# NVIDIA-NeMo/NeMo

Hardware: AMD Instinct MI355X
Metric: audio-sec/s training throughput, Conformer-CTC-Large @ 1/2/4/8 MI355X (higher is better)
Workload: dtype bf16; 1 GPU; Conformer-CTC-Large bf16, batch=32x20s synthetic 16 kHz clips per GPU, 1xMI355X (BASELINE.json configs[1]); global_batch=32, parallelism=dp1

## Files before the change

include/mi355x_asr.h:

```cpp
#ifndef MI355X_ASR_H
#define MI355X_ASR_H
#ifdef __cplusplus
extern "C" {
#endif

#define MI355X_DT_F32 0
#define MI355X_DT_BF16 1

enum {
  MI355X_EPI_STORE = 0,
  MI355X_EPI_SWISH_DROP = 1,
  MI355X_EPI_RESID = 2,
  MI355X_EPI_DSWISH = 3,
  MI355X_EPI_RELU_MASK = 4,
  MI355X_EPI_MUL_POS = 5,
  MI355X_EPI_SWISH_DROP_G = 6,
  MI355X_EPI_DSWISH_G = 7
};
typedef struct mi355x_gemm_desc {
  const void* A; const void* B; void* C;
  int M, N, K;
  long long lda, ldb, ldc;
  long long c_col_stride;
  int transA, transB;
// ... 227 lines not shown

int mi355x_adamw_step(void* params, const void* grads, void* exp_avg, void* exp_avg_sq, long long n, float lr, float beta1,
                      float beta2, float eps, float weight_decay, int step, float grad_scale, void* stream);
int mi355x_adamw_step_ex(void* params, const void* grads, void* exp_avg, void* exp_avg_sq, long long n, float lr, float beta1,
                         float beta2, float eps, float weight_decay, int step, float grad_scale, const void* clip_coef,
                         void* ema, float ema_decay, void* stream);
int mi355x_grad_sumsq(const void* grads, long long n, void* out_f64, void* stream);
int mi355x_clip_coef(const void* sumsq_f64, int nbuf, float scale, float max_norm, void* coef_f32x2, void* stream);
typedef struct mi355x_pack_entry {
  const void* src; void* dst;
  int rows, cols, nr2, nc2;
  long long sr1, sr2, sc1, sc2, pitch;
  long long tile_begin;
} mi355x_pack_entry;
int mi355x_pack_weights(const void* table_dev, int n_entries, long long total_tiles, int out_dtype, void* stream);
int mi355x_fill_f32(void* p, long long n, float value, void* stream);

const char* mi355x_asr_version(void);

int mi355x_set_step_counter(const void* dev_word);
int mi355x_set_null_launch(int on);

int mi355x_stream_create(int priority, void** out_stream);
int mi355x_stream_destroy(void* stream);
typedef struct mi355x_tape mi355x_tape;
int mi355x_tape_log_begin(void* origin_stream);
int mi355x_tape_log_end(void);
int mi355x_tape_from_graph(void* hip_graph, int max_lanes, mi355x_tape** out);
int mi355x_tape_replay(mi355x_tape* tape, void* stream, int join);
int mi355x_tape_join(mi355x_tape* tape, void* stream);
// ... 132 lines not shown
```

nemo_amd/_lib.py:

```python
from __future__ import annotations

import ctypes as C
import os

import torch

_HERE = os.path.dirname(os.path.abspath(__file__))
LIB_PATH = os.environ.get("MI355X_ASR_LIB", os.path.join(_HERE, "lib", "libmi355x_asr.so"))

vp, i32, i64, f32, f64, u32 = C.c_void_p, C.c_int, C.c_longlong, C.c_float, C.c_double, C.c_uint


class GemmDesc(C.Structure):
    _fields_ = [
        ("A", vp), ("B", vp), ("C", vp),
        ("M", i32), ("N", i32), ("K", i32),
        ("lda", i64), ("ldb", i64), ("ldc", i64), ("c_col_stride", i64),
        ("transA", i32), ("transB", i32),
        ("in_dtype", i32), ("c_dtype", i32),
        ("batch", i32), ("nb0", i32),
        ("sA0", i64), ("sA1", i64), ("sB0", i64), ("sB1", i64), ("sC0", i64), ("sC1", i64),
        ("bias", vp), ("alpha", f32),
        ("epilogue", i32), ("atomic", i32), ("splitk", i32),
        ("aux_in", vp), ("aux_in_dtype", i32),
# ... 12 lines not shown


class RowMap(C.Structure):
    _fields_ = [("nI", i32), ("nJ", i32), ("OI", i32), ("OJ", i32), ("si", i32), ("sj", i32), ("oi", i32), ("oj", i32)]


class FfnPackEntry(C.Structure):
    _fields_ = [("src", vp), ("k512", vp), ("kchunk", vp), ("d_ff", i32), ("is_w2", i32)]


class PackEntry(C.Structure):
    _fields_ = [
        ("src", vp), ("dst", vp),
        ("rows", i32), ("cols", i32), ("nr2", i32), ("nc2", i32),
        ("sr1", i64), ("sr2", i64), ("sc1", i64), ("sc2", i64), ("pitch", i64),
        ("tile_begin", i64),
    ]


SIGNATURES = {
    "mi355x_gemm": [C.POINTER(GemmDesc), vp],
    "mi355x_gemm_grouped": [C.POINTER(GemmDesc), i32, vp],
    "mi355x_gemm_config": [i32, i32],
    "mi355x_gemm_plan": [C.POINTER(GemmDesc), C.POINTER(i32 * 8)],
    "mi355x_set_step_counter": [vp],
    "mi355x_set_null_launch": [i32],
    "mi355x_ffn_fwd": [vp, i64, vp, vp, vp, vp, vp, i64, vp, i64, vp, i64, i32, i32, i32, f32, u32, u32, f32, u32, u32, f32, vp],
    "mi355x_ffn_pack": [vp, i32, i32, vp],
    "mi355x_ffn_bwd_dgrad": [vp, i64, vp, vp, vp, i64, vp, vp, vp, i64, i32, i32, i32, u32, u32, f32, vp],
    "mi355x_logmel_fwd": [vp, vp, vp, i32, i32, i32, vp, vp, vp, vp, i32, f32, f32, u32, f32, vp, i32, i32, i32, vp],
# ... 70 lines not shown
    "mi355x_bn_finalize_dev_count": [vp, vp, vp, vp, vp, vp, f32, f32, i32, vp],
    "mi355x_bn_eval_stats": [vp, vp, vp, vp, f32, i32, vp],
    "mi355x_bn_swish_fwd": [vp, vp, vp, vp, vp, vp, i32, i64, i32, vp],
    "mi355x_bn_swish_bwd_reduce": [vp, vp, vp, vp, vp, vp, vp, vp, vp, i32, i64, i32, vp, i64, vp],
    "mi355x_bn_stats_swish_fwd": [vp, vp, f64, vp, vp, vp, vp, vp, vp, vp, vp, f32, f32, i32, i64, i32, vp],
    "mi355x_bn_swish_bwd_apply": [vp, vp, vp, vp, vp, vp, vp, f64, i32, vp, i32, i64, i32, vp],
    "mi355x_bn_swish_bwd_apply_dev_count": [vp, vp, vp, vp, vp, vp, vp, vp, i32, vp, i32, i64, i32, vp],
    "mi355x_bn_param_grad": [vp, vp, vp, i32, vp],
    "mi355x_ctc_loss": [vp, vp, vp, vp, vp, vp, vp, vp, i32, i32, i32, i32, i32, f32, i32, vp],
    "mi355x_row_scale": [vp, vp, i64, i64, vp],
    "mi355x_adamw_step": [vp, vp, vp, vp, i64, f32, f32, f32, f32, f32, i32, f32, vp],
    "mi355x_adamw_step_ex": [vp, vp, vp, vp, i64, f32, f32, f32, f32, f32, i32, f32, vp, vp, f32, vp],
    "mi355x_grad_sumsq": [vp, i64, vp, vp],
    "mi355x_clip_coef": [vp, i32, f32, f32, vp, vp],
    "mi355x_pack_weights": [vp, i32, i64, i32, vp],
    "mi355x_fill_f32": [vp, i64, f32, vp],
    "mi355x_rnnt_workspace_elems": [i32, i32, i32, vp],
    "mi355x_rnnt_loss": [vp, vp, vp, vp, i32, i32, i32, i32, i32, f32, f32, f32, vp, vp, vp, i64, vp],
    "mi355x_rnnt_greedy_decode": [vp, i32, i64, vp, vp, vp, i64, vp, i64, vp, vp, vp, i64, vp, vp, i64, vp, i32, i32, i32, i32, i32,
                                  i32, i32, i32, vp, vp, vp, vp, i32, vp, vp, vp],
    "mi355x_dwconv_config": [i32],
    "mi355x_ctc_config": [i32],
    "mi355x_ctc_align_config": [i32],
    "mi355x_logmel_config": [i32],
    "mi355x_stream_create": [i32, vp],
    "mi355x_stream_destroy": [vp],
    "mi355x_tape_log_begin": [vp],
    "mi355x_tape_log_end": [],
    "mi355x_tape_from_graph": [vp, i32, vp],
    "mi355x_tape_replay": [vp, vp, i32],
# ... 70 lines not shown
```

nemo_amd/csrc/optim.hip:

```cpp
#include "common.h"
#include "mi355x_asr.h"

__global__ __launch_bounds__(256) void adamw_kernel(float* __restrict__ p, const float* __restrict__ g, float* __restrict__ m,
                                                    float* __restrict__ v, long long n4, float lr, float beta1, float beta2,
                                                    float eps, float wd, float bc1, float bc2_sqrt, float grad_scale,
                                                    const float* __restrict__ gclip, float* __restrict__ ema, float ema_decay) {
  const float gs = gclip ? grad_scale * gclip[0] : grad_scale;
  for (long long i = blockIdx.x * 256LL + threadIdx.x; i < n4; i += (long long)gridDim.x * 256) {
    float pp[4], gg[4], mm[4], vv[4];
    ld4(p + i * 4, pp); ld4(g + i * 4, gg); ld4(m + i * 4, mm); ld4(v + i * 4, vv);
#pragma unroll
    for (int j = 0; j < 4; ++j) {
      const float gr = gg[j] * gs;
      pp[j] *= (1.f - lr * wd);
      mm[j] = beta1 * mm[j] + (1.f - beta1) * gr;
      vv[j] = beta2 * vv[j] + (1.f - beta2) * gr * gr;
      const float denom = sqrtf(vv[j]) / bc2_sqrt + eps;
      pp[j] -= (lr / bc1) * (mm[j] / denom);
    }
    st4(p + i * 4, pp); st4(m + i * 4, mm); st4(v + i * 4, vv);
    if (ema) {
      float ee[4];
      ld4(ema + i * 4, ee);
#pragma unroll
      for (int j = 0; j < 4; ++j) ee[j] = ee[j] * ema_decay + (1.f - ema_decay) * pp[j];
      st4(ema + i * 4, ee);
    }
  }
}
__global__ __launch_bounds__(256) void sumsq_kernel(const float* __restrict__ g, long long n4, double* __restrict__ out) {
  __shared__ float red[8];
  float a = 0.f;
  for (long long i = blockIdx.x * 256LL + threadIdx.x; i < n4; i += (long long)gridDim.x * 256) {
    float x[4];
    ld4(g + i * 4, x);
    a += (x[0] * x[0] + x[1] * x[1]) + (x[2] * x[2] + x[3] * x[3]);
  }
  a = block_sum(a, red);
  if (threadIdx.x == 0) atomicAdd(out, (double)a);
}
__global__ void clip_coef_kernel(const double* __restrict__ sumsq, int nbuf, float scale, float max_norm, float* __restrict__ coef) {
  double t = 0.0;
  for (int i = 0; i < nbuf; ++i) t += sumsq[i];
  const float norm = scale * (float)sqrt(t);
  const float c = max_norm / (norm + 1e-6f);
  coef[0] = c < 1.f ? c : 1.f;
  coef[1] = norm;
}

struct PackEntry {
  const float* src; void* dst;
  int rows, cols, nr2, nc2;
  long long sr1, sr2, sc1, sc2, pitch;
  long long tile_begin;
};
#define PK_T 64
__global__ __launch_bounds__(256) void pack_kernel(const PackEntry* __restrict__ tab, int n_entries, int out_dt) {
  __shared__ float tile[PK_T][PK_T + 1];
  int lo = 0, hi = n_entries - 1;
  const long long bid = blockIdx.x;
  while (lo < hi) {
    const int mid = (lo + hi + 1) >> 1;
    if (tab[mid].tile_begin <= bid) lo = mid; else hi = mid - 1;
  }
  const PackEntry e = tab[lo];
  const int tiles_c = (e.cols + PK_T - 1) / PK_T;
  const int local = (int)(bid - e.tile_begin);
  const int tr = local / tiles_c, tc = local - tr * tiles_c;
  const bool col_fast = (e.sc2 == 1 && e.nc2 > 1) || (e.nc2 == 1 && e.sc1 == 1);
  const bool plain = e.nr2 == 1 && e.nc2 == 1;
  const long long fast_stride = col_fast ? e.sc1 : e.sr1, slow_stride = col_fast ? e.sr1 : e.sc1;
// ... 68 lines not shown
}
extern "C" int mi355x_adamw_step(void* params, const void* grads, void* exp_avg, void* exp_avg_sq, long long n, float lr,
                                 float beta1, float beta2, float eps, float weight_decay, int step, float grad_scale,
                                 void* stream) {
  mi_clear_errors();
  return adamw_launch(params, grads, exp_avg, exp_avg_sq, n, lr, beta1, beta2, eps, weight_decay, step, grad_scale, nullptr,
                      nullptr, 0.f, stream);
}
extern "C" int mi355x_adamw_step_ex(void* params, const void* grads, void* exp_avg, void* exp_avg_sq, long long n, float lr,
                                    float beta1, float beta2, float eps, float weight_decay, int step, float grad_scale,
                                    const void* clip_coef, void* ema, float ema_decay, void* stream) {
  mi_clear_errors();
  return adamw_launch(params, grads, exp_avg, exp_avg_sq, n, lr, beta1, beta2, eps, weight_decay, step, grad_scale, clip_coef,
                      ema, ema_decay, stream);
}
extern "C" int mi355x_grad_sumsq(const void* grads, long long n, void* out_f64, void* stream) {
  mi_clear_errors();
  if (!grads || !out_f64 || n <= 0 || (n & 3)) return MI_ERR_ARG;
  long long nb = ((n >> 2) + 255) / 256;
  if (nb > 2048) nb = 2048;
  MI_LAUNCH(sumsq_kernel, dim3((unsigned)nb), dim3(256), 0, (hipStream_t)stream, (const float*)grads, n >> 2,
                     (double*)out_f64);
  return mi_check_launch();
}
extern "C" int mi355x_clip_coef(const void* sumsq_f64, int nbuf, float scale, float max_norm, void* coef_f32x2, void* stream) {
  mi_clear_errors();
  if (!sumsq_f64 || !coef_f32x2 || nbuf <= 0 || !(max_norm > 0.f)) return MI_ERR_ARG;
  MI_LAUNCH(clip_coef_kernel, dim3(1), dim3(1), 0, (hipStream_t)stream, (const double*)sumsq_f64, nbuf, scale, max_norm,
                     (float*)coef_f32x2);
  return mi_check_launch();
// ... 19 lines not shown
```

nemo_amd/flat.py:

```python
from __future__ import annotations

from typing import Dict, List, Tuple

import torch
from torch import nn

ALIGN = 64


class FlatParams:
    def __init__(self, module: nn.Module, tail=None):
        self.module = module
        self._tail = tail or (lambda name: False)
        self.flat: torch.Tensor = None
        self.grad: torch.Tensor = None
        self.offsets: Dict[str, Tuple[int, int]] = {}
        self.order: List[str] = []
        self.generation = 0

    def _params(self):
        ps = [(n, p) for n, p in self.module.named_parameters() if p.dtype == torch.float32]
        return [x for x in ps if not self._tail(x[0])] + [x for x in ps if self._tail(x[0])]

    def is_valid(self) -> bool:
        if self.flat is None:
            return False
        base, gbase = self.flat.data_ptr(), self.grad.data_ptr()
        for n, p in self._params():
            off = self.offsets.get(n)
            if off is None or p.data_ptr() != base + off[0] * 4:
                return False
            if p.grad is None or p.grad.data_ptr() != gbase + off[0] * 4:
                return False
# ... 12 lines not shown
            total += (p.numel() + ALIGN - 1) // ALIGN * ALIGN
        flat = torch.zeros(total, dtype=torch.float32, device=device)
        grad = torch.zeros(total, dtype=torch.float32, device=device)
        with torch.no_grad():
            for n, p in params:
                off, num = self.offsets[n]
                view = flat[off: off + num].view(p.shape)
                view.copy_(p.data.to(device))
                gview = grad[off: off + num].view(p.shape)
                if p.grad is not None:
                    gview.copy_(p.grad.to(device))
                p.data = view
                p.grad = gview
        self.flat, self.grad = flat, grad
        self.generation += 1

    def ensure(self, device=None) -> None:
        if not self.is_valid():
            self.build(device)

    def range_of(self, prefix: str) -> Tuple[int, int]:
        names = [n for n in self.order if n.startswith(prefix) and not self._tail(n)]
        if not names:
            raise KeyError(prefix)
        start = min(self.offsets[n][0] for n in names)
        end = max((self.offsets[n][0] + self.offsets[n][1] + ALIGN - 1) // ALIGN * ALIGN for n in names)
        return start, end

    def tail_range(self) -> Tuple[int, int]:
        names = [n for n in self.order if self._tail(n)]
# ... 33 lines not shown
```

nemo_amd/modules/conformer_encoder.py:

```python
from __future__ import annotations

import math
import os
from collections import OrderedDict
from typing import Any, NamedTuple, Optional

import torch
from torch import nn

from .. import ops
from ..core import (AcousticEncodedRepresentation, BoolType, ChannelType, LengthsType, NeuralModule, NeuralType, SpectrogramType,
                    typecheck)
from ..flat import FlatParams
from ..packing import PackPlan

INF_VAL = 10000.0


def _pad8(n):
    return (n + 7) // 8 * 8


class _FeedForward(nn.Module):
    def __init__(self, d_model, d_ff, use_bias=True):
# ... 337 lines not shown
        self._wg_pending, self._wg_rows = None, None
        self._defer_flush = None
        self.conv2_implicit = os.environ.get("MI355X_CONV2_IMPLICIT", "1") != "0"
        self.fuse_bn_dwconv_bwd = os.environ.get("MI355X_BN_DW_FUSE", "1") != "0"
        self.fuse_glu_dwconv_bwd = os.environ.get("MI355X_GLU_DW_FUSE", "1") != "0"
        self.tap_reduce_side = os.environ.get("MI355X_TAP_REDUCE_SIDE", "1") != "0"
        self.pad_tile_skip = os.environ.get("MI355X_PAD_SKIP", "1") != "0"
        self.fuse_glu_dwconv_fwd = os.environ.get("MI355X_GLU_DW_FUSE_FWD", "1") != "0"
        self.ln_cast_fuse = os.environ.get("MI355X_LN_CAST_FUSE", "1") != "0"
        self.ffn_fused = os.environ.get("MI355X_FFN_FUSED", "0") != "0"
        self.swish_g = os.environ.get("MI355X_SWISH_G", "1") != "0"
        self._saving = False
        self.dpos_side_stream = os.environ.get("MI355X_DPOS_STREAM", "1") != "0"
        self.sub_wgrad_side_stream = os.environ.get("MI355X_SUB_WGRAD_STREAM", "1") != "0"
        self._plans = {}
        self._ws = {}
        self._ws_retired = []
        self._pos_cache = {}
        self._step_seed = 0
        self._weights_version = -1
        self._token = None
        _g = os.environ.get("MI355X_GRAPHS", "auto")
        self.use_graphs = _g != "0"
        self.graph_auto = _g not in ("0", "1", "2")
        self.graph_tape = os.environ.get("MI355X_TAPE", "1") != "0"
        self.graph_bwd_live = os.environ.get("MI355X_GRAPHS_BWD_LIVE", "0") != "0"
        self.graph_warmup = 2
        self.graph_trials = 4
        self.max_graph_sets = int(os.environ.get("MI355X_GRAPH_SETS", "64"))
        self.graph_warmup_inherited = 1
# ... 13 lines not shown
        self._step_word = None

    def set_max_audio_length(self, max_audio_length):
        self.max_audio_length = max_audio_length

    def update_max_seq_length(self, seq_length: int, device):
        if seq_length > self.max_audio_length:
            self.set_max_audio_length(seq_length)

    def flat_parameters(self) -> FlatParams:
        self._flatp.ensure()
        return self._flatp

    def weights_updated(self):
        self._weights_version += 1

    def load_state_dict(self, *a, **k):
        r = super().load_state_dict(*a, **k)
        self.weights_updated()
        return r

    @staticmethod
    def _calc_att_context(att_context_size, att_context_probs, att_context_style):
        if att_context_style not in ("regular", "chunked_limited"):
            raise ValueError(f"att_context_style={att_context_style}")
        if att_context_size:
            all_ = [list(x) for x in ([att_context_size] if isinstance(list(att_context_size)[0], int) else list(att_context_size))]
            for i, cs in enumerate(all_):
                if att_context_style == "chunked_limited":
                    if cs[0] > 0 and cs[0] % (cs[1] + 1) > 0:
# ... 187 lines not shown

    def _buf(self, name, shape, dtype, device, zero=False):
        n = 1
        for k in shape:
            n *= int(k)
        key = (name, dtype)
        t = self._ws.get(key)
        if t is None or t.device != device or t.numel() < n:
            cap = n if t is None or t.device != device else max(n, int(t.numel() * 1.25))
            if t is not None:
                self._ws_retired.append(t)
            t = torch.zeros(cap, dtype=dtype, device=device) if zero else torch.empty(cap, dtype=dtype, device=device)
            self._ws[key] = t
        return t[:n].view(shape)

    def _plan(self, cdt, device):
        key = (cdt, str(device), self._flatp.generation, self._geometry(cdt))
        plan = self._plans.get(key)
        if plan is None:
            self._plans = {}
            p = PackPlan(cdt, device)
            pf = PackPlan(torch.float32, device)
            srcs = []
            pe = self.pre_encode
            C_, F2 = pe._conv_channels, pe._feat_after
            if self.subsampling == "striding":
                p.add_conv3x3("pre.w2", pe.conv[2].weight.data); p.add_conv3x3("pre.w2t", pe.conv[2].weight.data, transpose=True)
                w2flat = pe.conv[2].weight.data.view(-1)
                for par_t in (0, 1):
                    for par_f in (0, 1):
                        slots = self._dgrad_slots(par_t, par_f, pe._pad)
# ... 38 lines not shown
                            p.add_block(f"L{i}.att.wqkvt", w.view(-1)[h * dk * d_:], d_, dk, col_off=j * dA + h * dkp, sr1=1, sc1=d_)
                        p.add_block(f"L{i}.att.wpos", a.linear_pos.weight.data.view(-1)[h * dk * d_:], dk, d_, row_off=h * dkp,
                                    sr1=d_, sc1=1)
                        p.add_block(f"L{i}.att.wo", wo.view(-1)[h * dk:], d_, dk, col_off=h * dkp, sr1=d_, sc1=1)
                        p.add_block(f"L{i}.att.wot", wo.view(-1)[h * dk:], dk, d_, row_off=h * dkp, sr1=1, sc1=d_)
                        for j, b in enumerate((a.linear_q.bias.data, a.linear_k.bias.data, a.linear_v.bias.data)):
                            pf.add_block(f"L{i}.att.bqkv", b[h * dk:], 1, dk, col_off=j * dA + h * dkp, sr1=0, sc1=1)
                        pf.add_block(f"L{i}.att.bu", a.pos_bias_u.data.view(-1)[h * dk:], 1, dk, col_off=h * dkp, sr1=0, sc1=1)
                        pf.add_block(f"L{i}.att.bv", a.pos_bias_v.data.view(-1)[h * dk:], 1, dk, col_off=h * dkp, sr1=0, sc1=1)
                c = L.conv
                p.add_matrix(f"L{i}.conv.pw1", c.pointwise_conv1.weight.data); p.add_matrix(f"L{i}.conv.pw1t", c.pointwise_conv1.weight.data, True)
                p.add_matrix(f"L{i}.conv.pw2", c.pointwise_conv2.weight.data); p.add_matrix(f"L{i}.conv.pw2t", c.pointwise_conv2.weight.data, True)
            p.finalize(); pf.finalize()
            plan = (p, pf, None, -2)
            self._plans[key] = plan
        if plan[3] != self._weights_version or self._force_pack:
            plan[0].run(); plan[1].run()
            plan = (plan[0], plan[1], plan[2], self._weights_version)
            self._plans[key] = plan
        return plan[0], plan[1]

    def _eager_point(self, fn):
        if self._capture is None:
            fn()
        else:
            self._capture.cut(fn)

    def _hook(self, lo, hi):
        self._eager_point(lambda: self.grad_ready_hook(lo, hi) if self.grad_ready_hook is not None else None)

    def _graph_key(self, mel, length):
        return (tuple(mel.shape), self._cdt(), str(mel.device), self._flatp.generation, self._syncbn_world(),
                self.grad_ready_hook is not None, self._wgrad_join_per_layer, self.wgrad_side_stream, self.wgrad_grouped,
                self.dpos_side_stream, self.sub_wgrad_side_stream, self.conv2_implicit, self.ln_cast_fuse, self.fuse_bn_dwconv_bwd, self.fuse_glu_dwconv_bwd, self.fuse_glu_dwconv_fwd, self.tap_reduce_side, self.pad_tile_skip,
                self.use_flash_attention, self.flash_delta_residual, self.syncbn_profile is not None, self.graph_tape, self.swish_g, self.dropout, self.dropout_att, self.dropout_emb, self.dropout_pre_encoder,
# ... 55 lines not shown
            for k2, g2 in self._graph_sets.items():
                if g2 is not gs and g2.decided is not None and not g2.inherited and k2[1:] == key[1:]:
                    gs.decided, gs.inherited = g2.decided, True
                    gs.samples = {"eager": [], "graph": []}
                    if gs.decided == "eager":
                        gs.fwd = gs.bwd = gs.S = gs.out = gs.enc_len = gs.mel = gs.dout = None
                    break
        if auto and gs.decided is None and self._dp_world() > 1:
            gs.decided = "eager"
        if auto and (gs.decided == "eager" or not self._in_step):
            self.live_steps += 1
            return None
        if gs.failed or gs.calls <= (self.graph_warmup_inherited if gs.inherited else self.graph_warmup):
            self.live_steps += 1
            return None
        if gs.fwd is None:
            try:
                self._capture_forward(gs, mel, length)
            except Exception as e:
                if os.environ.get("MI355X_GRAPHS") == "2":
                    raise
                import warnings
                warnings.warn(f"recording the encoder forward as hipGraphs failed ({type(e).__name__}: {e}); this shape keeps "
                              "running on the eager sequencer")
                gs.failed, gs.fwd, gs.S = True, None, None
                self.live_steps += 1
                return None
        elif auto and gs.decided is None and gs.bwd is not None:
            n_e, n_g = len(gs.samples["eager"]), len(gs.samples["graph"])
            if n_e >= self.graph_trials and n_g >= self.graph_trials:
# ... 1232 lines not shown
```

nemo_amd/ops.py:

```python
from __future__ import annotations

import contextlib
import ctypes as C
from typing import Optional

import torch

from ._lib import ConvGather, GemmDesc, PackEntry, RowMap, check, lib

F32, BF16 = 0, 1
EPI_STORE, EPI_SWISH_DROP, EPI_RESID, EPI_DSWISH, EPI_RELU_MASK, EPI_MUL_POS, EPI_SWISH_DROP_G, EPI_DSWISH_G = range(8)

_DT = {torch.float32: F32, torch.bfloat16: BF16}


def dt(t) -> int:
    try:
        return _DT[t.dtype if isinstance(t, torch.Tensor) else t]
    except KeyError:
        raise ValueError(f"unsupported dtype {t.dtype if isinstance(t, torch.Tensor) else t}")


def _ptr(t: Optional[torch.Tensor]) -> int:
    if t is None:
# ... 804 lines not shown
def row_scale(x, vec, rows, cols):
    check(lib.mi355x_row_scale(_ptr(x), _ptr(vec), rows, cols, _stream()), "row_scale")


def adamw_step(params, grads, exp_avg, exp_avg_sq, lr, beta1, beta2, eps, weight_decay, step, grad_scale=1.0,
               clip_coef=None, ema=None, ema_decay=0.0):
    if clip_coef is None and ema is None:
        check(lib.mi355x_adamw_step(_ptr(params), _ptr(grads), _ptr(exp_avg), _ptr(exp_avg_sq), params.numel(), lr, beta1,
                                    beta2, eps, weight_decay, step, grad_scale, _stream()), "adamw_step")
    else:
        check(lib.mi355x_adamw_step_ex(_ptr(params), _ptr(grads), _ptr(exp_avg), _ptr(exp_avg_sq), params.numel(), lr, beta1,
                                       beta2, eps, weight_decay, step, grad_scale, _ptr(clip_coef), _ptr(ema), ema_decay,
                                       _stream()), "adamw_step_ex")


def grad_sumsq(grads, out_f64):
    check(lib.mi355x_grad_sumsq(_ptr(grads), grads.numel(), _ptr(out_f64), _stream()), "grad_sumsq")


def clip_coef(sumsq_f64, scale, max_norm, coef):
    check(lib.mi355x_clip_coef(_ptr(sumsq_f64), int(sumsq_f64.numel()), float(scale), float(max_norm), _ptr(coef), _stream()),
          "clip_coef")



def pack_weights(table_dev, n_entries, total_tiles, out_dtype):
    check(lib.mi355x_pack_weights(_ptr(table_dev), n_entries, total_tiles, out_dtype, _stream()), "pack_weights")


def fill_f32(t, value=0.0):
# ... 19 lines not shown
```

nemo_amd/optim.py:

```python
from __future__ import annotations

from typing import List

import torch

from . import ops
import math

from .flat import FlatParams


class NoamAnnealing:
    def __init__(self, base_lr: float, d_model: int, warmup_steps=None, warmup_ratio=None, max_steps=None, min_lr=0.0):
        assert not (warmup_steps is not None and warmup_ratio is not None), "Either use particular number of step or ratio"
        assert warmup_ratio is None or max_steps is not None, "If there is a ratio, there should be a total steps"
        if base_lr < min_lr:
            raise ValueError("initial learning rate lower than the minimum learning rate")
        self._normalize = d_model ** (-0.5)
        self.base_lr, self.min_lr = base_lr, min_lr
        self.warmup_steps = warmup_steps if warmup_steps is not None else (int(warmup_ratio * max_steps) if warmup_ratio else 0)
        self.last_epoch = 0

    def lr_at(self, step: int) -> float:
        step = max(1, step)
# ... 130 lines not shown
    def _ema_of(self, fp: FlatParams):
        if self.ema_decay is None:
            return None
        key = (id(fp), fp.generation)
        e = self._ema.get(key)
        if e is None:
            old = [v for k, v in self._ema.items() if k[0] == id(fp)]
            if old and old[0].numel() == fp.flat.numel():
                e = old[0].to(fp.flat.device)
            else:
                e = fp.flat.detach().clone()
            self._ema = {k: v for k, v in self._ema.items() if k[0] != id(fp)}
            self._ema[key] = e
        return e

    def zero_grad(self):
        for fp in self.flats:
            fp.ensure()
            fp.zero_grad()

    def begin_step(self, lr: float = None, grad_scale: float = 1.0):
        self.step_count += 1
        self._cur = (self.lr if lr is None else lr, grad_scale)
        self._done = {id(fp): [] for fp in self.flats}
        for fp in self.flats:
            fp.ensure()
            self._moments(fp)
            self._ema_of(fp)
        return self.max_grad_norm is None

    def step_range(self, fp: FlatParams, lo: int, hi: int):
        if getattr(self, "_cur", None) is None or self.max_grad_norm is not None or hi <= lo:
            return
        lr, grad_scale = self._cur
        m, v = self._moments(fp)
        ema = self._ema_of(fp)
        for tlo, thi in fp.trainable_ranges():
            a, b = max(lo, tlo), min(hi, thi)
            if a >= b:
                continue
            ops.adamw_step(fp.flat[a:b], fp.grad[a:b], m[a:b], v[a:b], lr, self.betas[0], self.betas[1], self.eps,
                           self.weight_decay, self.step_count, grad_scale, ema=None if ema is None else ema[a:b],
                           ema_decay=self.ema_decay or 0.0)
        self._done[id(fp)].append((lo, hi))

    def finish_step(self):
        lr, grad_scale = self._cur
        for fp in self.flats:
            done = sorted(self._done[id(fp)])
            pos, rest = 0, []
            for lo, hi in done:
                if lo > pos:
                    rest.append((pos, lo))
                pos = max(pos, hi)
            if pos < fp.flat.numel():
                rest.append((pos, fp.flat.numel()))
            for lo, hi in rest:
                self.step_range(fp, lo, hi)
        self._cur = None
        for fp in self.flats:
            if hasattr(fp.module, "weights_updated"):
                fp.module.weights_updated()

    def step(self, lr: float = None, grad_scale: float = 1.0):
        self.step_count += 1
        lr = self.lr if lr is None else lr
        coef = None
        if self.max_grad_norm:
            dev = self.flats[0].flat.device
            if self._clip is None or self._clip[0].device != dev:
                self._clip = (torch.zeros(len(self.flats), dtype=torch.float64, device=dev),
                              torch.zeros(2, dtype=torch.float32, device=dev))
            sumsq, coef = self._clip
            sumsq.zero_()
            for i, fp in enumerate(self.flats):
                for lo, hi in fp.trainable_ranges():
                    ops.grad_sumsq(fp.grad[lo:hi], sumsq[i:i + 1])
            ops.clip_coef(sumsq, grad_scale, self.max_grad_norm, coef)
            self.last_grad_norm = coef[1:2]
        for fp in self.flats:
            m, v = self._moments(fp)
            ema = self._ema_of(fp)
            for lo, hi in fp.trainable_ranges():
                ops.adamw_step(fp.flat[lo:hi], fp.grad[lo:hi], m[lo:hi], v[lo:hi], lr, self.betas[0], self.betas[1], self.eps,
                               self.weight_decay, self.step_count, grad_scale, clip_coef=coef,
                               ema=None if ema is None else ema[lo:hi], ema_decay=self.ema_decay or 0.0)
        for fp in self.flats:
            if hasattr(fp.module, "weights_updated"):
                fp.module.weights_updated()

    def swap_ema_weights(self):
        import contextlib

        @contextlib.contextmanager
        def ctx():
            if self.ema_decay is None:
                yield
                return
            pairs = [(fp, self._ema_of(fp)) for fp in self.flats]

            def swap():
# ... 31 lines not shown
```

nemo_amd/packing.py:

```python
from __future__ import annotations

import ctypes as C
from typing import Dict, List, Tuple

import numpy as np
import torch

from . import ops
from ._lib import PackEntry


def _pad8(n: int) -> int:
    return (n + 7) // 8 * 8


class PackPlan:
    def __init__(self, dtype: torch.dtype, device):
        self.dtype = dtype
        self.device = torch.device(device)
        self._images: Dict[str, Tuple[int, int, int]] = {}
        self._pending: List[tuple] = []
        self._size = 0
        self.arena = None
        self._table = None
        self._n = 0
        self._tiles = 0
        self._views: Dict[str, torch.Tensor] = {}
        self._ffn: List[tuple] = []
        self._ffn_table = None

    def new_image(self, name: str, rows: int, cols: int) -> None:
        pitch = _pad8(cols)
        self._images[name] = (self._size, rows, pitch)
        self._size += (rows * pitch + 63) // 64 * 64

    def add_block(self, name: str, src: torch.Tensor, rows: int, cols: int, *, row_off=0, col_off=0, nr2=1, nc2=1,
                  sr1=0, sr2=0, sc1=0, sc2=0) -> None:
        assert src.dtype == torch.float32 and src.is_contiguous()
        self._pending.append((name, src, rows, cols, row_off, col_off, nr2, nc2, sr1, sr2, sc1, sc2))

    def add_matrix(self, name: str, w: torch.Tensor, transpose: bool = False):
        R, Cc = w.shape[0], int(np.prod(w.shape[1:]))
        if not transpose:
            self.new_image(name, R, Cc)
# ... 40 lines not shown
            self.add_block(name, w, F_ * C_, d, nr2=C_, nc2=1, sr1=1, sr2=F_, sc1=C_ * F_)
        return name

    def add_ffn(self, prefix: str, w1: torch.Tensor, w2: torch.Tensor) -> None:
        dff = w1.shape[0]
        assert self.dtype == torch.bfloat16 and tuple(w1.shape) == (dff, 512) and tuple(w2.shape) == (512, dff) and dff % 64 == 0
        assert w1.dtype == torch.float32 and w2.dtype == torch.float32 and w1.is_contiguous() and w2.is_contiguous()
        for nm in ("w1p", "w1tp", "w2p", "w2tp"):
            self.new_image(f"{prefix}.{nm}", dff // 2, 1024)
        self._ffn.append((prefix, w1, w2, dff))

    def finalize(self) -> None:
        self.arena = torch.zeros(max(self._size, 64), dtype=self.dtype, device=self.device)
        es = self.arena.element_size()
        base = self.arena.data_ptr()
        entries = (PackEntry * len(self._pending))()
        tiles = 0
        for i, (name, src, rows, cols, ro, co, nr2, nc2, sr1, sr2, sc1, sc2) in enumerate(self._pending):
            off, irows, pitch = self._images[name]
            assert ro + rows <= irows and co + cols <= pitch, name
            e = entries[i]
            e.src = src.data_ptr()
            assert co % 8 == 0, name
            e.dst = base + (off + ro * pitch + co) * es
            e.rows, e.cols, e.nr2, e.nc2 = rows, cols, nr2, nc2
            e.sr1, e.sr2, e.sc1, e.sc2, e.pitch = sr1, sr2, sc1, sc2, pitch
            e.tile_begin = tiles
            tiles += ((rows + 63) // 64) * ((cols + 63) // 64)
        raw = bytes(entries)
        self._table = torch.frombuffer(bytearray(raw), dtype=torch.uint8).to(self.device) if raw else None
        self._n, self._tiles = len(self._pending), tiles
        self._srcs = [p[1] for p in self._pending]
        if self._ffn:
            from ._lib import FfnPackEntry
            fe = (FfnPackEntry * (2 * len(self._ffn)))()
            for i, (prefix, w1, w2, dff) in enumerate(self._ffn):
                off = {nm: self._images[f"{prefix}.{nm}"][0] for nm in ("w1p", "w1tp", "w2p", "w2tp")}
                a, b = fe[2 * i], fe[2 * i + 1]
                a.src, a.k512, a.kchunk, a.d_ff, a.is_w2 = w1.data_ptr(), base + off["w1p"] * es, base + off["w1tp"] * es, dff, 0
                b.src, b.k512, b.kchunk, b.d_ff, b.is_w2 = w2.data_ptr(), base + off["w2tp"] * es, base + off["w2p"] * es, dff, 1
            self._ffn_table = torch.frombuffer(bytearray(bytes(fe)), dtype=torch.uint8).to(self.device)
            self._srcs += [t for f in self._ffn for t in (f[1], f[2])]
        for name, (off, rows, pitch) in self._images.items():
            self._views[name] = self.arena[off: off + rows * pitch].view(rows, pitch)

    def source_ptrs(self):
        return [s.data_ptr() for s in self._srcs]

    def run(self) -> None:
        if self._n:
            ops.pack_weights(self._table, self._n, self._tiles, ops.dt(self.dtype))
        if self._ffn:
            ops.ffn_pack(self._ffn_table, 2 * len(self._ffn), max(f[3] for f in self._ffn))

    def __getitem__(self, name: str) -> torch.Tensor:
        return self._views[name]

    def pitch(self, name: str) -> int:
        return self._images[name][2]
```

Measured before the change: 18280 audio-sec/s.

## Fuse AdamW update with bf16 weight packing for plain matrix parameters

Adds a fused AdamW kernel that updates fp32 parameters and also writes the bf16 packed weight images (plain or transposed) for simple matrix parameters straight from the updated values. The separate pack pass then only handles the remaining entries. Bookkeeping tracks whether every covered matrix was handled by the fused path, with a catch-up pack when it was not. The aim is to save a separate read of the fp32 weights and a kernel launch per step. The cost is more complex cross-module state tracking and transposed stores that are not coalesced.

```diff
diff --git a/include/mi355x_asr.h b/include/mi355x_asr.h
--- a/include/mi355x_asr.h
+++ b/include/mi355x_asr.h
@@ -265,6 +265,18 @@
   long long tile_begin;
 } mi355x_pack_entry;
 int mi355x_pack_weights(const void* table_dev, int n_entries, long long total_tiles, int out_dtype, void* stream);
+typedef struct mi355x_adamw_pack_entry {
+  long long off;
+  int rows, cols;
+  void* dst0; void* dst1;
+  long long pitch0, pitch1;
+  int trans0, trans1;
+  long long tile_begin;
+} mi355x_adamw_pack_entry;
+int mi355x_adamw_pack_step(const void* table_dev, int n_entries, long long tile_base, long long n_tiles, void* params,
+                           const void* grads, void* exp_avg, void* exp_avg_sq, long long lo, long long hi, float lr, float beta1,
+                           float beta2, float eps, float weight_decay, int step, float grad_scale, const void* clip_coef,
+                           void* ema, float ema_decay, void* stream);
 int mi355x_fill_f32(void* p, long long n, float value, void* stream);
 
 const char* mi355x_asr_version(void);
diff --git a/nemo_amd/_lib.py b/nemo_amd/_lib.py
--- a/nemo_amd/_lib.py
+++ b/nemo_amd/_lib.py
@@ -50,6 +50,15 @@
         ("src", vp), ("dst", vp),
         ("rows", i32), ("cols", i32), ("nr2", i32), ("nc2", i32),
         ("sr1", i64), ("sr2", i64), ("sc1", i64), ("sc2", i64), ("pitch", i64),
+        ("tile_begin", i64),
+    ]
+
+
+class AdamwPackEntry(C.Structure):
+    _fields_ = [
+        ("off", i64), ("rows", i32), ("cols", i32),
+        ("dst0", vp), ("dst1", vp), ("pitch0", i64), ("pitch1", i64),
+        ("trans0", i32), ("trans1", i32),
         ("tile_begin", i64),
     ]
 
@@ -150,6 +159,7 @@
     "mi355x_grad_sumsq": [vp, i64, vp, vp],
     "mi355x_clip_coef": [vp, i32, f32, f32, vp, vp],
     "mi355x_pack_weights": [vp, i32, i64, i32, vp],
+    "mi355x_adamw_pack_step": [vp, i32, i64, i64, vp, vp, vp, vp, i64, i64, f32, f32, f32, f32, f32, i32, f32, vp, vp, f32, vp],
     "mi355x_fill_f32": [vp, i64, f32, vp],
     "mi355x_rnnt_workspace_elems": [i32, i32, i32, vp],
     "mi355x_rnnt_loss": [vp, vp, vp, vp, i32, i32, i32, i32, i32, f32, f32, f32, vp, vp, vp, i64, vp],
diff --git a/nemo_amd/csrc/optim.hip b/nemo_amd/csrc/optim.hip
--- a/nemo_amd/csrc/optim.hip
+++ b/nemo_amd/csrc/optim.hip
@@ -1,30 +1,146 @@
 #include "common.h"
 #include "mi355x_asr.h"
+
+#define PK_T 64
+struct AdamwC { float lr, beta1, beta2, eps, wd, bc1, bc2_sqrt, gs; };
+__device__ __forceinline__ void adamw_update(float& pp, const float gg, float& mm, float& vv, const AdamwC& c) {
+  const float gr = gg * c.gs;
+  mm = __builtin_fmaf(c.beta1, mm, (1.f - c.beta1) * gr);
+  vv = __builtin_fmaf(c.beta2, vv, gr * ((1.f - c.beta2) * gr));
+  const float denom = sqrtf(vv) / c.bc2_sqrt + c.eps;
+  const float upd = -(c.lr / c.bc1) * (mm / denom);
+  pp = __builtin_fmaf(__builtin_fmaf(-c.lr, c.wd, 1.f), pp, upd);
+}
+__device__ __forceinline__ float ema_update(const float ee, const float pp, const float ema_decay) {
+  return __builtin_fmaf(ema_decay, ee, (1.f - ema_decay) * pp);
+}
+__device__ __forceinline__ void adamw_compute4(float (&pp)[4], const float (&gg)[4], float (&mm)[4], float (&vv)[4],
+                                               const AdamwC& c) {
+#pragma unroll
+  for (int j = 0; j < 4; ++j) adamw_update(pp[j], gg[j], mm[j], vv[j], c);
+}
+__device__ __forceinline__ void adamw_update4(float* __restrict__ p, const float* __restrict__ g, float* __restrict__ m,
+                                              float* __restrict__ v, float* __restrict__ ema, float ema_decay, long long i,
+                                              const AdamwC& c, float (&pp)[4]) {
+  float gg[4], mm[4], vv[4];
+  ld4(p + i, pp); ld4(g + i, gg); ld4(m + i, mm); ld4(v + i, vv);
+  adamw_compute4(pp, gg, mm, vv, c);
+  st4(p + i, pp); st4(m + i, mm); st4(v + i, vv);
+  if (ema) {
+    float ee[4];
+    ld4(ema + i, ee);
+#pragma unroll
+    for (int j = 0; j < 4; ++j) ee[j] = ema_update(ee[j], pp[j], ema_decay);
+    st4(ema + i, ee);
+  }
+}
 
 __global__ __launch_bounds__(256) void adamw_kernel(float* __restrict__ p, const float* __restrict__ g, float* __restrict__ m,
                                                     float* __restrict__ v, long long n4, float lr, float beta1, float beta2,
                                                     float eps, float wd, float bc1, float bc2_sqrt, float grad_scale,
                                                     const float* __restrict__ gclip, float* __restrict__ ema, float ema_decay) {
-  const float gs = gclip ? grad_scale * gclip[0] : grad_scale;
+  const AdamwC c = {lr, beta1, beta2, eps, wd, bc1, bc2_sqrt, gclip ? grad_scale * gclip[0] : grad_scale};
   for (long long i = blockIdx.x * 256LL + threadIdx.x; i < n4; i += (long long)gridDim.x * 256) {
-    float pp[4], gg[4], mm[4], vv[4];
-    ld4(p + i * 4, pp); ld4(g + i * 4, gg); ld4(m + i * 4, mm); ld4(v + i * 4, vv);
-#pragma unroll
-    for (int j = 0; j < 4; ++j) {
-      const float gr = gg[j] * gs;
-      pp[j] *= (1.f - lr * wd);
-      mm[j] = beta1 * mm[j] + (1.f - beta1) * gr;
-      vv[j] = beta2 * vv[j] + (1.f - beta2) * gr * gr;
-      const float denom = sqrtf(vv[j]) / bc2_sqrt + eps;
-      pp[j] -= (lr / bc1) * (mm[j] / denom);
-    }
-    st4(p + i * 4, pp); st4(m + i * 4, mm); st4(v + i * 4, vv);
-    if (ema) {
-      float ee[4];
-      ld4(ema + i * 4, ee);
-#pragma unroll
-      for (int j = 0; j < 4; ++j) ee[j] = ee[j] * ema_decay + (1.f - ema_decay) * pp[j];
-      st4(ema + i * 4, ee);
+    float pp[4];
+    adamw_update4(p, g, m, v, ema, ema_decay, i * 4, c, pp);
+  }
+}
+
+#define APK_CHUNK 4096
+typedef mi355x_adamw_pack_entry AdamwPackEntry;
+__global__ __launch_bounds__(256) void adamw_pack_kernel(const AdamwPackEntry* __restrict__ tab, int n_entries, long long tile_base,
+                                                         float* __restrict__ p, const float* __restrict__ g,
+                                                         float* __restrict__ m, float* __restrict__ v, long long lo_el,
+                                                         long long hi_el, float lr, float beta1, float beta2, float eps, float wd,
+                                                         float bc1, float bc2_sqrt, float grad_scale,
+                                                         const float* __restrict__ gclip, float* __restrict__ ema,
+                                                         float ema_decay) {
+  const AdamwC c = {lr, beta1, beta2, eps, wd, bc1, bc2_sqrt, gclip ? grad_scale * gclip[0] : grad_scale};
+  int lo = 0, hi = n_entries - 1;
+  const long long bid = tile_base + blockIdx.x;
+  while (lo < hi) {
+    const int mid = (lo + hi + 1) >> 1;
+    if (tab[mid].tile_begin <= bid) lo = mid; else hi = mid - 1;
+  }
+  const AdamwPackEntry e = tab[lo];
+  const int local = (int)(bid - e.tile_begin);
+  if (e.rows == 0) {
+    long long a = e.off + (long long)local * APK_CHUNK, b = a + APK_CHUNK;
+    if (b > e.off + e.cols) b = e.off + e.cols;
+    if (a < lo_el) a = lo_el;
+    if (b > hi_el) b = hi_el;
+    for (long long i = a + threadIdx.x * 4; i < b; i += 256 * 4) {
+      float pp[4];
+      adamw_update4(p, g, m, v, ema, ema_decay, i, c, pp);
+    }
+    return;
+  }
+  const int tiles_c = (e.cols + PK_T - 1) / PK_T;
+  const int tr = local / tiles_c, tc = local - tr * tiles_c;
+  const int rb = tr * PK_T + (threadIdx.x >> 4) * 4, cc = tc * PK_T + (threadIdx.x & 15) * 4;
+  const bool vec = !(e.cols & 3);
+  float np[4][4];
+#pragma unroll
+  for (int k = 0; k < 4; ++k) {
+    const int r = rb + k;
+    const int nv = (r < e.rows && cc < e.cols) ? (e.cols - cc < 4 ? e.cols - cc : 4) : 0;
+    const bool whole = vec && nv == 4;
+    const long long i = e.off + (long long)r * e.cols + cc;
+    float pp[4] = {0.f, 0.f, 0.f, 0.f}, gg[4] = {0.f, 0.f, 0.f, 0.f}, mm[4] = {0.f, 0.f, 0.f, 0.f}, vv[4] = {0.f, 0.f, 0.f, 0.f};
+    float ee[4] = {0.f, 0.f, 0.f, 0.f};
+    if (whole) {
+      ld4(p + i, pp); ld4(g + i, gg); ld4(m + i, mm); ld4(v + i, vv);
+      if (ema) ld4(ema + i, ee);
+    } else {
+#pragma unroll
+      for (int j = 0; j < 4; ++j)
+        if (j < nv) {
+          pp[j] = p[i + j]; gg[j] = g[i + j]; mm[j] = m[i + j]; vv[j] = v[i + j];
+          if (ema) ee[j] = ema[i + j];
+        }
+    }
+    adamw_compute4(pp, gg, mm, vv, c);
+#pragma unroll
+    for (int j = 0; j < 4; ++j) ee[j] = ema_update(ee[j], pp[j], ema_decay);
+    if (whole) {
+      st4(p + i, pp); st4(m + i, mm); st4(v + i, vv);
+      if (ema) st4(ema + i, ee);
+    } else {
+#pragma unroll
+      for (int j = 0; j < 4; ++j) {
+        if (j < nv) {
+          p[i + j] = pp[j]; m[i + j] = mm[j]; v[i + j] = vv[j];
+          if (ema) ema[i + j] = ee[j];
+        } else {
+          pp[j] = 0.f;
+        }
+      }
+    }
+#pragma unroll
+    for (int j = 0; j < 4; ++j) np[k][j] = pp[j];
+  }
+  const int rows8 = (e.rows + 7) & ~7, cols8 = (e.cols + 7) & ~7;
+#pragma unroll
+  for (int d = 0; d < 2; ++d) {
+    bf16_t* dst = (bf16_t*)(d ? e.dst1 : e.dst0);
+    if (!dst) continue;
+    const long long pitch = d ? e.pitch1 : e.pitch0;
+    if (!(d ? e.trans1 : e.trans0)) {
+      if (cc < cols8) {
+#pragma unroll
+        for (int k = 0; k < 4; ++k)
+          if (rb + k < e.rows)
+            *reinterpret_cast<uint2*>(dst + (long long)(rb + k) * pitch + cc) =
+                make_uint2(pack_bf2(np[k][0], np[k][1]), pack_bf2(np[k][2], np[k][3]));
+      }
+    } else {
+      if (rb < rows8) {
+#pragma unroll
+        for (int j = 0; j < 4; ++j)
+          if (cc + j < e.cols)
+            *reinterpret_cast<uint2*>(dst + (long long)(cc + j) * pitch + rb) =
+                make_uint2(pack_bf2(np[0][j], np[1][j]), pack_bf2(np[2][j], np[3][j]));
+      }
     }
   }
 }
@@ -54,7 +170,6 @@
   long long sr1, sr2, sc1, sc2, pitch;
   long long tile_begin;
 };
-#define PK_T 64
 __global__ __launch_bounds__(256) void pack_kernel(const PackEntry* __restrict__ tab, int n_entries, int out_dt) {
   __shared__ float tile[PK_T][PK_T + 1];
   int lo = 0, hi = n_entries - 1;
@@ -153,6 +268,21 @@
   return adamw_launch(params, grads, exp_avg, exp_avg_sq, n, lr, beta1, beta2, eps, weight_decay, step, grad_scale, clip_coef,
                       ema, ema_decay, stream);
 }
+extern "C" int mi355x_adamw_pack_step(const void* table_dev, int n_entries, long long tile_base, long long n_tiles, void* params,
+                                      const void* grads, void* exp_avg, void* exp_avg_sq, long long lo, long long hi, float lr,
+                                      float beta1, float beta2, float eps, float weight_decay, int step, float grad_scale,
+                                      const void* clip_coef, void* ema, float ema_decay, void* stream) {
+  mi_clear_errors();
+  if (!table_dev || n_entries <= 0 || tile_base < 0 || n_tiles <= 0 || n_tiles > 0x7fffffffLL) return MI_ERR_ARG;
+  if (!params || !grads || !exp_avg || !exp_avg_sq || lo < 0 || hi <= lo || (lo & 3) || (hi & 3) || step < 1) return MI_ERR_ARG;
+  if (ema && !(ema_decay >= 0.f && ema_decay <= 1.f)) return MI_ERR_ARG;
+  const float bc1 = 1.f - powf(beta1, (float)step);
+  const float bc2s = sqrtf(1.f - powf(beta2, (float)step));
+  MI_LAUNCH(adamw_pack_kernel, dim3((unsigned)n_tiles), dim3(256), 0, (hipStream_t)stream, (const AdamwPackEntry*)table_dev,
+                     n_entries, tile_base, (float*)params, (const float*)grads, (float*)exp_avg, (float*)exp_avg_sq, lo, hi, lr,
+                     beta1, beta2, eps, weight_decay, bc1, bc2s, grad_scale, (const float*)clip_coef, (float*)ema, ema_decay);
+  return mi_check_launch();
+}
 extern "C" int mi355x_grad_sumsq(const void* grads, long long n, void* out_f64, void* stream) {
   mi_clear_errors();
   if (!grads || !out_f64 || n <= 0 || (n & 3)) return MI_ERR_ARG;
diff --git a/nemo_amd/flat.py b/nemo_amd/flat.py
--- a/nemo_amd/flat.py
+++ b/nemo_amd/flat.py
@@ -17,6 +17,19 @@
         self.offsets: Dict[str, Tuple[int, int]] = {}
         self.order: List[str] = []
         self.generation = 0
+        self.fused_table = None
+
+    def set_fused_table(self, table) -> None:
+        self.fused_table = table
+
+    def fused(self):
+        t = self.fused_table
+        return t if t is not None and t.matches(self) else None
+
+    def fused_lookup(self, lo: int, hi: int):
+        t = self.fused()
+        sub = t.lookup(lo, hi) if t is not None else None
+        return None if sub is None else (t, sub)
 
     def _params(self):
         ps = [(n, p) for n, p in self.module.named_parameters() if p.dtype == torch.float32]
@@ -59,6 +72,7 @@
                 p.grad = gview
         self.flat, self.grad = flat, grad
         self.generation += 1
+        self.fused_table = None
 
     def ensure(self, device=None) -> None:
         if not self.is_valid():
diff --git a/nemo_amd/modules/conformer_encoder.py b/nemo_amd/modules/conformer_encoder.py
--- a/nemo_amd/modules/conformer_encoder.py
+++ b/nemo_amd/modules/conformer_encoder.py
@@ -375,6 +375,7 @@
         self.dpos_side_stream = os.environ.get("MI355X_DPOS_STREAM", "1") != "0"
         self.sub_wgrad_side_stream = os.environ.get("MI355X_SUB_WGRAD_STREAM", "1") != "0"
         self._plans = {}
+        self.adamw_pack = os.environ.get("MI355X_ADAMW_PACK", "1") != "0"
         self._ws = {}
         self._ws_retired = []
         self._pos_cache = {}
@@ -418,6 +419,9 @@
 
     def weights_updated(self):
         self._weights_version += 1
+        tab = self._flatp.fused_table
+        if tab is not None:
+            tab.plan.covered_at = self._weights_version if tab.take_complete() else None
 
     def load_state_dict(self, *a, **k):
         r = super().load_state_dict(*a, **k)
@@ -635,7 +639,7 @@
             self._ws[key] = t
         return t[:n].view(shape)
 
-    def _plan(self, cdt, device):
+    def _plan(self, cdt, device, pack=True):
         key = (cdt, str(device), self._flatp.generation, self._geometry(cdt))
         plan = self._plans.get(key)
         if plan is None:
@@ -704,11 +708,33 @@
             p.finalize(); pf.finalize()
             plan = (p, pf, None, -2)
             self._plans[key] = plan
+            fused_ok = cdt == torch.bfloat16 and self._flatp.flat.device == p.arena.device
+            self._flatp.set_fused_table(p.build_fused(self._flatp) if fused_ok else None)
+        if plan[0].fused is not None:
+            plan[0].fused.enabled = self.adamw_pack
+        if not pack:
+            return plan[0], plan[1]
         if plan[3] != self._weights_version or self._force_pack:
-            plan[0].run(); plan[1].run()
+            p = plan[0]
+            rest_only = p.fused is not None and p.covered_at == self._weights_version
+            p.run(rest_only=rest_only); plan[1].run()
+            if p.fused is not None:
+                p.covered_at = self._weights_version
             plan = (plan[0], plan[1], plan[2], self._weights_version)
             self._plans[key] = plan
         return plan[0], plan[1]
+
+    def _covered_catch_up(self, cdt, device):
+        plan = self._plans.get((cdt, str(device), self._flatp.generation, self._geometry(cdt)))
+        if plan is None:
+            return
+        p = plan[0]
+        if p.fused is None:
+            return
+        p.fused.enabled = self.adamw_pack
+        if p.covered_at != self._weights_version:
+            p.run(covered_only=True)
+            p.covered_at = self._weights_version
 
     def _eager_point(self, fn):
         if self._capture is None:
@@ -794,6 +820,7 @@
         if gs.failed or gs.calls <= (self.graph_warmup_inherited if gs.inherited else self.graph_warmup):
             self.live_steps += 1
             return None
+        self._covered_catch_up(self._cdt(), mel.device)
         if gs.fwd is None:
             try:
                 self._capture_forward(gs, mel, length)
diff --git a/nemo_amd/ops.py b/nemo_amd/ops.py
--- a/nemo_amd/ops.py
+++ b/nemo_amd/ops.py
@@ -6,7 +6,7 @@
 
 import torch
 
-from ._lib import ConvGather, GemmDesc, PackEntry, RowMap, check, lib
+from ._lib import AdamwPackEntry, ConvGather, GemmDesc, PackEntry, RowMap, check, lib
 
 F32, BF16 = 0, 1
 EPI_STORE, EPI_SWISH_DROP, EPI_RESID, EPI_DSWISH, EPI_RELU_MASK, EPI_MUL_POS, EPI_SWISH_DROP_G, EPI_DSWISH_G = range(8)
@@ -842,6 +842,18 @@
                                        _stream()), "adamw_step_ex")
 
 
+def adamw_pack_step(table_dev, first, n_entries, tile_base, n_tiles, params, grads, exp_avg, exp_avg_sq, lo, hi, lr, beta1, beta2,
+                    eps, weight_decay, step, grad_scale=1.0, clip_coef=None, ema=None, ema_decay=0.0):
+    if not (0 <= lo < hi <= params.numel()) or grads.numel() != params.numel() or exp_avg.numel() != params.numel() \
+            or exp_avg_sq.numel() != params.numel() or (ema is not None and ema.numel() != params.numel()):
+        raise ValueError("adamw_pack_step: range / buffer sizes")
+    if first < 0 or n_entries <= 0 or (first + n_entries) * C.sizeof(AdamwPackEntry) > table_dev.numel():
+        raise ValueError("adamw_pack_step: entry range")
+    check(lib.mi355x_adamw_pack_step(_ptr(table_dev) + first * C.sizeof(AdamwPackEntry), n_entries, tile_base, n_tiles, _ptr(params),
+                                     _ptr(grads), _ptr(exp_avg), _ptr(exp_avg_sq), lo, hi, lr, beta1, beta2, eps, weight_decay, step,
+                                     grad_scale, _ptr(clip_coef), _ptr(ema), ema_decay, _stream()), "adamw_pack_step")
+
+
 def grad_sumsq(grads, out_f64):
     check(lib.mi355x_grad_sumsq(_ptr(grads), grads.numel(), _ptr(out_f64), _stream()), "grad_sumsq")
 
diff --git a/nemo_amd/optim.py b/nemo_amd/optim.py
--- a/nemo_amd/optim.py
+++ b/nemo_amd/optim.py
@@ -168,6 +168,32 @@
             self._ema[key] = e
         return e
 
+    def _adamw(self, fp: FlatParams, a: int, b: int, m, v, ema, lr, grad_scale, clip_coef=None):
+        tab = fp.fused()
+        sub = tab.lookup(a, b) if tab is not None else None
+        if sub is not None:
+            first, n, tile_base, tiles, matrices = sub
+            ops.adamw_pack_step(tab.table, first, n, tile_base, tiles, fp.flat, fp.grad, m, v, a, b, lr, self.betas[0],
+                                self.betas[1], self.eps, self.weight_decay, self.step_count, grad_scale, clip_coef=clip_coef,
+                                ema=ema, ema_decay=self.ema_decay or 0.0)
+            tab.note(matrices)
+            return
+        if tab is not None:
+            tab.note_fallback()
+        ops.adamw_step(fp.flat[a:b], fp.grad[a:b], m[a:b], v[a:b], lr, self.betas[0], self.betas[1], self.eps,
+                       self.weight_decay, self.step_count, grad_scale, clip_coef=clip_coef,
+                       ema=None if ema is None else ema[a:b], ema_decay=self.ema_decay or 0.0)
+
+    def _fused_begin(self):
+        for fp in self.flats:
+            if fp.fused_table is not None:
+                fp.fused_table.begin()
+
+    def _fused_end(self):
+        for fp in self.flats:
+            if fp.fused_table is not None:
+                fp.fused_table.end()
+
     def zero_grad(self):
         for fp in self.flats:
             fp.ensure()
@@ -177,6 +203,7 @@
         self.step_count += 1
         self._cur = (self.lr if lr is None else lr, grad_scale)
         self._done = {id(fp): [] for fp in self.flats}
+        self._fused_begin()
         for fp in self.flats:
             fp.ensure()
             self._moments(fp)
@@ -193,9 +220,7 @@
             a, b = max(lo, tlo), min(hi, thi)
             if a >= b:
                 continue
-            ops.adamw_step(fp.flat[a:b], fp.grad[a:b], m[a:b], v[a:b], lr, self.betas[0], self.betas[1], self.eps,
-                           self.weight_decay, self.step_count, grad_scale, ema=None if ema is None else ema[a:b],
-                           ema_decay=self.ema_decay or 0.0)
+            self._adamw(fp, a, b, m, v, ema, lr, grad_scale)
         self._done[id(fp)].append((lo, hi))
 
     def finish_step(self):
@@ -212,6 +237,7 @@
             for lo, hi in rest:
                 self.step_range(fp, lo, hi)
         self._cur = None
+        self._fused_end()
         for fp in self.flats:
             if hasattr(fp.module, "weights_updated"):
                 fp.module.weights_updated()
@@ -219,6 +245,7 @@
     def step(self, lr: float = None, grad_scale: float = 1.0):
         self.step_count += 1
         lr = self.lr if lr is None else lr
+        self._fused_begin()
         coef = None
         if self.max_grad_norm:
             dev = self.flats[0].flat.device
@@ -236,9 +263,8 @@
             m, v = self._moments(fp)
             ema = self._ema_of(fp)
             for lo, hi in fp.trainable_ranges():
-                ops.adamw_step(fp.flat[lo:hi], fp.grad[lo:hi], m[lo:hi], v[lo:hi], lr, self.betas[0], self.betas[1], self.eps,
-                               self.weight_decay, self.step_count, grad_scale, clip_coef=coef,
-                               ema=None if ema is None else ema[lo:hi], ema_decay=self.ema_decay or 0.0)
+                self._adamw(fp, lo, hi, m, v, ema, lr, grad_scale, coef)
+        self._fused_end()
         for fp in self.flats:
             if hasattr(fp.module, "weights_updated"):
                 fp.module.weights_updated()
diff --git a/nemo_amd/packing.py b/nemo_amd/packing.py
--- a/nemo_amd/packing.py
+++ b/nemo_amd/packing.py
@@ -7,11 +7,68 @@
 import torch
 
 from . import ops
-from ._lib import PackEntry
+from ._lib import AdamwPackEntry, PackEntry
 
 
 def _pad8(n: int) -> int:
     return (n + 7) // 8 * 8
+
+
+LINEAR_CHUNK = 4096
+
+
+class FusedTable:
+
+    def __init__(self, plan, fp, table, entries, tile_begin, covered):
+        self.plan, self.table = plan, table
+        self.flat_ptr, self.numel, self.generation = fp.flat.data_ptr(), fp.flat.numel(), fp.generation
+        self.entries = entries
+        self.tile_begin = tile_begin
+        self.covered = covered
+        self.starts = [e[0] for e in entries]
+        self.n_matrices = sum(1 for e in entries if e[1])
+        self._cache = {}
+        self._seen, self._fallback, self._complete = 0, False, False
+        self.enabled = True
+
+    def matches(self, fp) -> bool:
+        return self.enabled and fp.flat is not None and fp.generation == self.generation and fp.flat.data_ptr() == self.flat_ptr \
+            and fp.flat.numel() == self.numel
+
+    def lookup(self, lo: int, hi: int):
+        key = (lo, hi)
+        r = self._cache.get(key, 0)
+        if r != 0:
+            return r
+        r = None
+        if 0 <= lo < hi <= self.numel and not (lo & 3) and not (hi & 3):
+            import bisect
+            i0 = bisect.bisect_right(self.starts, lo) - 1
+            i1 = bisect.bisect_left(self.starts, hi)
+            first, last = self.entries[i0], self.entries[i1 - 1]
+            cut = (first[1] and first[0] < lo) or (last[1] and last[0] + last[1] * last[2] > hi)
+            if not cut:
+                r = (i0, i1 - i0, self.tile_begin[i0], self.tile_begin[i1] - self.tile_begin[i0],
+                     sum(1 for e in self.entries[i0:i1] if e[1]))
+        self._cache[key] = r
+        return r
+
+    def begin(self):
+        self._seen, self._fallback, self._complete = 0, False, False
+
+    def note(self, matrices: int):
+        self._seen += matrices
+
+    def note_fallback(self):
+        self._fallback = True
+
+    def end(self):
+        self._complete = not self._fallback and self._seen == self.n_matrices
+        self._seen, self._fallback = 0, False
+
+    def take_complete(self) -> bool:
+        c, self._complete = self._complete, False
+        return c
 
 
 class PackPlan:
@@ -28,6 +85,9 @@
         self._views: Dict[str, torch.Tensor] = {}
         self._ffn: List[tuple] = []
         self._ffn_table = None
+        self.fused = None
+        self.covered_at = None
+        self._rest = self._covered = None
 
     def new_image(self, name: str, rows: int, cols: int) -> None:
         pitch = _pad8(cols)
@@ -98,21 +158,7 @@
         self.arena = torch.zeros(max(self._size, 64), dtype=self.dtype, device=self.device)
         es = self.arena.element_size()
         base = self.arena.data_ptr()
-        entries = (PackEntry * len(self._pending))()
-        tiles = 0
-        for i, (name, src, rows, cols, ro, co, nr2, nc2, sr1, sr2, sc1, sc2) in enumerate(self._pending):
-            off, irows, pitch = self._images[name]
-            assert ro + rows <= irows and co + cols <= pitch, name
-            e = entries[i]
-            e.src = src.data_ptr()
-            assert co % 8 == 0, name
-            e.dst = base + (off + ro * pitch + co) * es
-            e.rows, e.cols, e.nr2, e.nc2 = rows, cols, nr2, nc2
-            e.sr1, e.sr2, e.sc1, e.sc2, e.pitch = sr1, sr2, sc1, sc2, pitch
-            e.tile_begin = tiles
-            tiles += ((rows + 63) // 64) * ((cols + 63) // 64)
-        raw = bytes(entries)
-        self._table = torch.frombuffer(bytearray(raw), dtype=torch.uint8).to(self.device) if raw else None
+        self._table, tiles = self._entry_table(range(len(self._pending)))
         self._n, self._tiles = len(self._pending), tiles
         self._srcs = [p[1] for p in self._pending]
         if self._ffn:
@@ -128,13 +174,108 @@
         for name, (off, rows, pitch) in self._images.items():
             self._views[name] = self.arena[off: off + rows * pitch].view(rows, pitch)
 
+    def _entry_table(self, idx):
+        idx = list(idx)
+        es, base = self.arena.element_size(), self.arena.data_ptr()
+        entries = (PackEntry * max(len(idx), 1))()
+        tiles = 0
+        for k, i in enumerate(idx):
+            name, src, rows, cols, ro, co, nr2, nc2, sr1, sr2, sc1, sc2 = self._pending[i]
+            off, irows, pitch = self._images[name]
+            assert ro + rows <= irows and co + cols <= pitch, name
+            e = entries[k]
+            e.src = src.data_ptr()
+            assert co % 8 == 0, name
+            e.dst = base + (off + ro * pitch + co) * es
+            e.rows, e.cols, e.nr2, e.nc2 = rows, cols, nr2, nc2
+            e.sr1, e.sr2, e.sc1, e.sc2, e.pitch = sr1, sr2, sc1, sc2, pitch
+            e.tile_begin = tiles
+            tiles += ((rows + 63) // 64) * ((cols + 63) // 64)
+        raw = bytes(entries)[: len(idx) * C.sizeof(PackEntry)]
+        return (torch.frombuffer(bytearray(raw), dtype=torch.uint8).to(self.device) if raw else None), tiles
+
+    def plain_maps(self):
+        out = []
+        if self.dtype != torch.bfloat16:
+            return out
+        for i, (name, src, rows, cols, ro, co, nr2, nc2, sr1, sr2, sc1, sc2) in enumerate(self._pending):
+            if nr2 != 1 or nc2 != 1:
+                continue
+            if sc1 == 1 and sr1 == cols:
+                out.append((i, src.data_ptr(), rows, cols, 0))
+            elif sr1 == 1 and sc1 == rows:
+                out.append((i, src.data_ptr(), cols, rows, 1))
+        return out
+
+    def build_fused(self, fp):
+        assert self.arena is not None, "finalize() first"
+        base, numel = fp.flat.data_ptr(), fp.flat.numel()
+        groups = {}
+        for i, ptr, R, Cc, tr in self.plain_maps():
+            d = ptr - base
+            if d < 0 or d % 16 or (R * Cc) % 4 or d // 4 + R * Cc > numel or R < 1 or Cc < 1:
+                continue
+            groups.setdefault((d // 4, R, Cc), []).append((i, tr))
+        mats, end = [], 0
+        for (off, R, Cc), dsts in sorted(groups.items()):
+            if len(dsts) > 2 or off < end:
+                continue
+            mats.append((off, R, Cc, dsts))
+            end = off + R * Cc
+        if not mats or fp.flat.device != self.device:
+            return None
+        es, abase = self.arena.element_size(), self.arena.data_ptr()
+        rows_ = []
+
+        def linear(a, b):
+            while a < b:
+                n = min(b - a, 1 << 30)
+                rows_.append((a, 0, n, []))
+                a += n
+        pos = 0
+        for off, R, Cc, dsts in mats:
+            linear(pos, off)
+            dd = []
+            for i, tr in dsts:
+                name, _, rows, cols, ro, co = self._pending[i][:6]
+                ioff, _, pitch = self._images[name]
+                dd.append((abase + (ioff + ro * pitch + co) * es, pitch, tr))
+            rows_.append((off, R, Cc, dd))
+            pos = off + R * Cc
+        linear(pos, numel)
+        ent = (AdamwPackEntry * len(rows_))()
+        tile_begin, tiles = [], 0
+        for k, (off, R, Cc, dd) in enumerate(rows_):
+            e = ent[k]
+            e.off, e.rows, e.cols = off, R, Cc
+            dd = dd + [(0, 0, 0)] * (2 - len(dd))
+            (e.dst0, e.pitch0, e.trans0), (e.dst1, e.pitch1, e.trans1) = dd[0], dd[1]
+            e.tile_begin = tiles
+            tile_begin.append(tiles)
+            tiles += ((R + 63) // 64) * ((Cc + 63) // 64) if R else (Cc + LINEAR_CHUNK - 1) // LINEAR_CHUNK
+        tile_begin.append(tiles)
+        covered = sorted(i for m in mats for i, _ in m[3])
+        cset = set(covered)
+        self._covered = self._entry_table(covered) + (len(covered),)
+        rest = [i for i in range(len(self._pending)) if i not in cset]
+        self._rest = self._entry_table(rest) + (len(rest),)
+        dev_table = torch.frombuffer(bytearray(bytes(ent)), dtype=torch.uint8).to(self.device)
+        self.fused = FusedTable(self, fp, dev_table, [(r[0], r[1], r[2]) for r in rows_], tile_begin, covered)
+        self.covered_at = None
+        return self.fused
+
     def source_ptrs(self):
         return [s.data_ptr() for s in self._srcs]
 
-    def run(self) -> None:
-        if self._n:
-            ops.pack_weights(self._table, self._n, self._tiles, ops.dt(self.dtype))
-        if self._ffn:
+    def run(self, rest_only: bool = False, covered_only: bool = False) -> None:
+        if self.fused is not None and (rest_only or covered_only):
+            table, tiles, n = self._covered if covered_only else self._rest
+        else:
+            assert not covered_only
+            table, tiles, n = self._table, self._tiles, self._n
+        if n:
+            ops.pack_weights(table, n, tiles, ops.dt(self.dtype))
+        if self._ffn and not covered_only:
             ops.ffn_pack(self._ffn_table, 2 * len(self._ffn), max(f[3] for f in self._ffn))
 
     def __getitem__(self, name: str) -> torch.Tensor:
```

Result: no change. 18350 audio-sec/s (median of 6 runs) (+0.4%).
